# PKU-VCL-Geometry/GeoSplatting

Measured on AMD Instinct MI355X. Metric: fwd+bwd views/sec at 2M Gaussians, 800x800, higher is better.
Workload: dtype f32

## Files before the change

geosplatting_amd/csrc/gs_sort.hip:

```cpp
#include "gs_common.h"

#include <cstdlib>
#include <cstring>

#define RS_THREADS 256
#define RS_WAVES 4
#define RS_ITEMS 8
#define RS_TILE (RS_THREADS * RS_ITEMS)
#define RS_WCHUNK (64 * RS_ITEMS)

typedef unsigned long long u64;

static int tile_bits(int tile_w, int tile_h)
{
    unsigned n = (unsigned)(tile_w * tile_h);
    int b = 0;
    while (n > 1) { n >>= 1; ++b; }
    return b + 1;
}

struct PairItem { u64 key; int32_t val; };
struct PairIn {
    const u64* keys; const int32_t* vals;
    __device__ __forceinline__ PairItem load(int64_t i) const { return PairItem{ keys[i], vals[i] }; }
};
struct PairOut {
    u64* keys; int32_t* vals;
    __device__ __forceinline__ void store(int64_t i, const PairItem& it) const { keys[i] = it.key; vals[i] = it.val; }
};
struct PairDigit {
    int shift; unsigned mask;
    __device__ __forceinline__ unsigned operator()(const PairItem& it) const { return (unsigned)(it.key >> shift) & mask; }
};

struct U2In {
    const uint2* p;
    __device__ __forceinline__ uint2 load(int64_t i) const { return p[i]; }
};
struct U2Out {
    uint2* p;
    __device__ __forceinline__ void store(int64_t i, const uint2& it) const { p[i] = it; }
};
struct DepthIn {
    const float* depths;
    __device__ __forceinline__ uint2 load(int64_t i) const { return make_uint2(__float_as_uint(depths[i]), (unsigned)i); }
};
struct XDigit {
    int shift; unsigned mask;
    __device__ __forceinline__ unsigned operator()(const uint2& it) const { return (it.x >> shift) & mask; }
};
struct FinalTiles {
    int32_t* tile_ids; int32_t* flatten_ids;
    __device__ __forceinline__ void store(int64_t i, const uint2& it) const
    {
        flatten_ids[i] = (int32_t)it.y;
        tile_ids[i] = (int32_t)it.x;
    }
};
struct FinalOut {
    u64* isect_ids; int32_t* flatten_ids; const float* depths;
    __device__ __forceinline__ void store(int64_t i, const uint2& it) const
    {
        flatten_ids[i] = (int32_t)it.y;
        isect_ids[i] = ((u64)it.x << 32) | (u64)__float_as_uint(depths[it.y]);
    }
};

template <typename Item, typename In, typename Digit>
__global__ void __launch_bounds__(RS_THREADS)
radix_hist_kernel(GsCount nc, In in, Digit digit, int nbins, int nblocks, unsigned* __restrict__ table)
{
    const int64_t n = gs_count(nc);
    __shared__ unsigned hist[256];
    hist[threadIdx.x] = 0u;
    __syncthreads();
    const int64_t base = (int64_t)blockIdx.x * RS_TILE;
#pragma unroll 4
    for (int k = 0; k < RS_ITEMS; ++k) {
        const int64_t i = base + (int64_t)k * RS_THREADS + threadIdx.x;
        if (i < n) atomicAdd(&hist[digit(in.load(i))], 1u);
    }
    __syncthreads();
    if ((int)threadIdx.x < nbins) table[(size_t)threadIdx.x * nblocks + blockIdx.x] = hist[threadIdx.x];
}

__global__ void __launch_bounds__(256)
radix_rowscan_kernel(int nblocks, unsigned* __restrict__ table, unsigned* __restrict__ row_total)
{
    __shared__ unsigned wsum[4];
    unsigned* row = table + (size_t)blockIdx.x * nblocks;
    const int lane = threadIdx.x & 63, wave = threadIdx.x >> 6;
    unsigned carry = 0u;
    for (int i0 = 0; i0 < nblocks; i0 += 256) {
        const int i = i0 + threadIdx.x;
        const unsigned v = i < nblocks ? row[i] : 0u;
        unsigned incl = v;
        incl = gs_wave_incl_scan(incl);
        if (lane == 63) wsum[wave] = incl;
        __syncthreads();
        unsigned before = 0u, all = 0u;
        for (int w = 0; w < 4; ++w) { if (w < wave) before += wsum[w]; all += wsum[w]; }
        if (i < nblocks) row[i] = carry + before + incl - v;
        carry += all;
        __syncthreads();
    }
    if (threadIdx.x == 0) row_total[blockIdx.x] = carry;
}

template <typename Item, typename In, typename Digit, typename Out, int NBITS>
__global__ void __launch_bounds__(RS_THREADS)
radix_scatter_kernel(GsCount nc, In in, Digit digit, int nblocks, const unsigned* __restrict__ table,
                     const unsigned* __restrict__ row_total, Out out)
{
    const int64_t n = gs_count(nc);
    constexpr int NB = 1 << NBITS;
    __shared__ unsigned cnt[RS_WAVES][NB];
    __shared__ unsigned dstart[NB];
    __shared__ unsigned gbase[NB];
    __shared__ Item stage[RS_TILE];
    const int lane = threadIdx.x & 63, wave = threadIdx.x >> 6;
    for (int i = threadIdx.x; i < RS_WAVES * NB; i += RS_THREADS) (&cnt[0][0])[i] = 0u;
    __syncthreads();
    const int64_t bbase = (int64_t)blockIdx.x * RS_TILE;
    const int64_t wbase = bbase + (int64_t)wave * RS_WCHUNK;
    const int n_here = (n - bbase) < RS_TILE ? (int)((n - bbase) > 0 ? (n - bbase) : 0) : RS_TILE;
    const u64 lane_lt = (1ull << lane) - 1ull;
    Item item[RS_ITEMS];
    unsigned dig[RS_ITEMS];
    unsigned rank[RS_ITEMS];
#pragma unroll
    for (int k = 0; k < RS_ITEMS; ++k) {
        const int64_t i = wbase + (int64_t)k * 64 + lane;
        const bool valid = i < n;
        if (valid) item[k] = in.load(i);
        const unsigned d = valid ? digit(item[k]) : 0u;
        u64 m = __ballot(valid);
#pragma unroll
        for (int b = 0; b < NBITS; ++b) {
            const bool bit = (d >> b) & 1u;
            const u64 bal = __ballot(bit);
            m &= bit ? bal : ~bal;
        }
        const unsigned old = cnt[wave][d];
        __builtin_amdgcn_wave_barrier();
        const unsigned r = __popcll(m & lane_lt);
        if (valid && r == 0u) cnt[wave][d] = old + (unsigned)__popcll(m);
        __builtin_amdgcn_fence(__ATOMIC_RELEASE, "wavefront");
        __builtin_amdgcn_wave_barrier();
        __builtin_amdgcn_fence(__ATOMIC_ACQUIRE, "wavefront");
        dig[k] = d;
        rank[k] = old + r;
    }
    __syncthreads();
    {
        const int d = threadIdx.x;
        unsigned tot = 0u;
        if (d < NB) for (int w = 0; w < RS_WAVES; ++w) tot += cnt[w][d];
        unsigned incl = tot;
        incl = gs_wave_incl_scan(incl);
        __shared__ unsigned wtot[RS_WAVES];
        if (lane == 63) wtot[wave] = incl;
        __syncthreads();
        unsigned before = 0u;
        for (int w = 0; w < wave; ++w) before += wtot[w];
        if (d < NB) dstart[d] = before + incl - tot;
        __syncthreads();
        const unsigned rt = d < NB ? row_total[d] : 0u;
        unsigned rincl = rt;
        rincl = gs_wave_incl_scan(rincl);
        if (lane == 63) wtot[wave] = rincl;
        __syncthreads();
        unsigned rbefore = 0u;
        for (int w = 0; w < wave; ++w) rbefore += wtot[w];
        if (d < NB) gbase[d] = rbefore + rincl - rt + table[(size_t)d * nblocks + blockIdx.x];
    }
    __syncthreads();
#pragma unroll
    for (int k = 0; k < RS_ITEMS; ++k) {
        const int64_t i = wbase + (int64_t)k * 64 + lane;
        if (i < n) {
            const unsigned d = dig[k];
            unsigned off = dstart[d] + rank[k];
            for (int w = 0; w < wave; ++w) off += cnt[w][d];
            stage[off] = item[k];
        }
    }
    __syncthreads();
#pragma unroll 4
    for (int k = 0; k < RS_ITEMS; ++k) {
        const int p = k * RS_THREADS + (int)threadIdx.x;
        if (p < n_here) {
            const Item it = stage[p];
            const unsigned d = digit(it);
            out.store((int64_t)gbase[d] + (int64_t)(p - (int)dstart[d]), it);
        }
    }
}

template <typename Item, typename In, typename Digit, typename Out>
static int radix_pass(GsCount nc, In in, Digit digit, Out out, int nbits, unsigned* table, hipStream_t s)
{
    const int64_t n = nc.n;
    const int nblocks = (int)((n + RS_TILE - 1) / RS_TILE);
    const int nbins = 1 << nbits;
    unsigned* row_total = table + (size_t)256 * nblocks;
    hipLaunchKernelGGL((radix_hist_kernel<Item, In, Digit>), dim3(nblocks), dim3(RS_THREADS), 0, s, nc, in, digit, nbins, nblocks, table);
    GS_CHECK_LAUNCH();
    hipLaunchKernelGGL(radix_rowscan_kernel, dim3(nbins), dim3(256), 0, s, nblocks, table, row_total);
    GS_CHECK_LAUNCH();
    switch (nbits) {
#define RS_CASE(B) case B: hipLaunchKernelGGL((radix_scatter_kernel<Item, In, Digit, Out, B>), dim3(nblocks), dim3(RS_THREADS), 0, s, nc, in, digit, nblocks, table, row_total, out); break;
        RS_CASE(1) RS_CASE(2) RS_CASE(3) RS_CASE(4) RS_CASE(5) RS_CASE(6) RS_CASE(7) RS_CASE(8)
#undef RS_CASE
        default: gs_set_error("radix_pass: bad digit width %d", nbits); return GS_EINVAL;
    }
    GS_CHECK_LAUNCH();
    return GS_OK;
}

static size_t align256(size_t x) { return (x + 255) & ~(size_t)255; }
static size_t table_bytes(int64_t n) { return align256(((size_t)256 * (size_t)((n + RS_TILE - 1) / RS_TILE + 1) + 512) * sizeof(unsigned)); }

extern "C" size_t gs_sort_ws_bytes(int64_t n_isects, int tile_w, int tile_h)
{
    if (n_isects <= 0) return 0;
    (void)tile_w; (void)tile_h;
    return table_bytes(n_isects) + align256((size_t)n_isects * 8) + align256((size_t)n_isects * 4) + 256;
}

extern "C" int gs_isect_sort(int64_t n_isects, const int64_t* isect_ids, const int32_t* flatten_ids,
                             int64_t* isect_ids_sorted, int32_t* flatten_ids_sorted, int tile_w, int tile_h,
                             void* ws, size_t ws_bytes, void* stream)
{
    GS_CHECK_ARG(n_isects >= 0 && tile_w > 0 && tile_h > 0, "bad sizes");
    if (n_isects == 0) return GS_OK;
    GS_CHECK_ARG(ws != nullptr, "workspace must not be NULL");
    if (ws_bytes < gs_sort_ws_bytes(n_isects, tile_w, tile_h)) { gs_set_error("gs_isect_sort: workspace too small"); return GS_ENOSPC; }
    hipStream_t s = (hipStream_t)stream;
    char* p = (char*)ws;
    unsigned* table = (unsigned*)p; p += table_bytes(n_isects);
    u64* tk = (u64*)p; p += align256((size_t)n_isects * 8);
    int32_t* tv = (int32_t*)p;
    const int end_bit = 32 + tile_bits(tile_w, tile_h);
    const int npass = (end_bit + 7) / 8;
    const u64* src_k = (const u64*)isect_ids; const int32_t* src_v = flatten_ids;
    for (int pass = 0; pass < npass; ++pass) {
        const int shift = pass * 8;
        const int nbits = (end_bit - shift) < 8 ? (end_bit - shift) : 8;
        const bool to_out = ((npass - 1 - pass) % 2) == 0;
        u64* dk = to_out ? (u64*)isect_ids_sorted : tk;
        int32_t* dv = to_out ? flatten_ids_sorted : tv;
        const int rc = radix_pass<PairItem>(GsCount{ n_isects, nullptr }, PairIn{ src_k, src_v }, PairDigit{ shift, (1u << nbits) - 1u }, PairOut{ dk, dv }, nbits, table, s);
        if (rc != GS_OK) return rc;
        src_k = dk; src_v = dv;
    }
    return GS_OK;
}

__device__ __forceinline__ void tile_range_sorted(float mx, float my, int radius, int tile_size, int tw, int th,
                                                  int& x0, int& y0, int& x1, int& y1)
{
#pragma clang fp contract(off)
    const float ts = (float)tile_size;
    const float tr = (float)radius / ts;
    const float tx = mx / ts, ty = my / ts;
    const float fx0 = floorf(tx - tr), fy0 = floorf(ty - tr);
    const float fx1 = ceilf(tx + tr), fy1 = ceilf(ty + tr);
    x0 = fx0 < 0.0f ? 0 : (fx0 > (float)tw ? tw : (int)fx0);
    y0 = fy0 < 0.0f ? 0 : (fy0 > (float)th ? th : (int)fy0);
    x1 = fx1 < 0.0f ? 0 : (fx1 > (float)tw ? tw : (int)fx1);
    y1 = fy1 < 0.0f ? 0 : (fy1 > (float)th ? th : (int)fy1);
}

#define EM_THREADS 256
#define EM_PER 4
#define EM_LOOK 4
#define EM_TILE (EM_THREADS * EM_PER)

__global__ void __launch_bounds__(256)
tile_rect_kernel(GsCount vc, const float* __restrict__ means2d, const int32_t* __restrict__ radii, int tile_size, int tile_w, int tile_h,
                 uint2* __restrict__ rect)
{
    const int V = (int)gs_count(vc);
    const int v = blockIdx.x * blockDim.x + threadIdx.x;
    if (v >= V) return;
    const float2 m = *reinterpret_cast<const float2*>(means2d + 2 * (size_t)v);
    int x0 = 0, y0 = 0, x1 = 0, y1 = 0;
    const int r = radii[v];
    if (r > 0) tile_range_sorted(m.x, m.y, r, tile_size, tile_w, tile_h, x0, y0, x1, y1);
    rect[v] = make_uint2((unsigned)x0 | ((unsigned)y0 << 16), (unsigned)x1 | ((unsigned)y1 << 16));
}
__device__ __forceinline__ unsigned rect_count(uint2 q)
{
    const int w = (int)(q.y & 0xffffu) - (int)(q.x & 0xffffu), h = (int)(q.y >> 16) - (int)(q.x >> 16);
    return (w > 0 && h > 0) ? (unsigned)(w * h) : 0u;
}

static size_t bf_state_bytes(int V) { return align256(16 + 2 * (size_t)((V + EM_TILE - 1) / EM_TILE + 1) * sizeof(u64)); }

extern "C" size_t gs_isect_bin_ws_bytes(int V, int64_t n_isects, int tile_w, int tile_h)
{
    (void)tile_w; (void)tile_h;
    const size_t v = V > 0 ? (size_t)V : 1, n = n_isects > 0 ? (size_t)n_isects : 1;
    const size_t tb = table_bytes((int64_t)(v > n ? v : n));
    return tb + 3 * align256(v * 8) + bf_state_bytes((int)v) + 2 * align256(n * 8) + 256;
}

__global__ void capacity_check_kernel(const long long* __restrict__ counts, long long v_cap, long long i_cap, long long* __restrict__ status)
{
    if (threadIdx.x != 0 || blockIdx.x != 0) return;
    const long long V = counts[0], I = counts[1];
    if (V > v_cap || I > i_cap) {
        status[0] = GS_ENOSPC;
        if (I > status[1]) status[1] = I;
        if (V > status[2]) status[2] = V;
    }
}

static int isect_bin_impl(int V, const float* means2d, const int32_t* radii, const float* depths, int64_t n_isects,
                          const long long* counts_dev, int tile_size, int tile_w, int tile_h, int64_t* isect_ids_sorted,
                          int32_t* flatten_ids_sorted, void* ws, size_t ws_bytes, void* stream, int32_t* tile_ids_sorted);

extern "C" int gs_isect_bin(int V, const float* means2d, const int32_t* radii, const float* depths,
                            const int32_t* tiles_per_gauss, int64_t n_isects, int tile_size, int tile_w, int tile_h,
                            int64_t* isect_ids_sorted, int32_t* flatten_ids_sorted, void* ws, size_t ws_bytes, void* stream)
{
    (void)tiles_per_gauss;
    return isect_bin_impl(V, means2d, radii, depths, n_isects, nullptr, tile_size, tile_w, tile_h, isect_ids_sorted, flatten_ids_sorted,
                          ws, ws_bytes, stream, nullptr);
}

extern "C" int gs_isect_bin_cap(int V_cap, const float* means2d, const int32_t* radii, const float* depths, const int64_t* counts_dev,
                                int64_t n_isects_cap, int tile_size, int tile_w, int tile_h, int64_t* isect_ids_sorted,
                                int32_t* flatten_ids_sorted, void* ws, size_t ws_bytes, int64_t* status_dev, void* stream)
{
    GS_CHECK_ARG(counts_dev != nullptr && status_dev != nullptr, "counts_dev / status_dev must not be NULL");
    hipLaunchKernelGGL(capacity_check_kernel, dim3(1), dim3(64), 0, (hipStream_t)stream, (const long long*)counts_dev, (long long)V_cap,
                       (long long)n_isects_cap, (long long*)status_dev);
    GS_CHECK_LAUNCH();
    return isect_bin_impl(V_cap, means2d, radii, depths, n_isects_cap, (const long long*)counts_dev, tile_size, tile_w, tile_h,
                          isect_ids_sorted, flatten_ids_sorted, ws, ws_bytes, stream, nullptr);
}

extern "C" int gs_isect_bin_tiles_cap(int V_cap, const float* means2d, const int32_t* radii, const float* depths, const int64_t* counts_dev,
                                      int64_t n_isects_cap, int tile_size, int tile_w, int tile_h, int32_t* tile_ids_sorted,
                                      int32_t* flatten_ids_sorted, void* ws, size_t ws_bytes, int64_t* status_dev, void* stream)
{
    GS_CHECK_ARG(counts_dev != nullptr && status_dev != nullptr && tile_ids_sorted != nullptr, "counts_dev / status_dev / tile_ids_sorted must not be NULL");
    hipLaunchKernelGGL(capacity_check_kernel, dim3(1), dim3(64), 0, (hipStream_t)stream, (const long long*)counts_dev, (long long)V_cap,
                       (long long)n_isects_cap, (long long*)status_dev);
    GS_CHECK_LAUNCH();
    return isect_bin_impl(V_cap, means2d, radii, depths, n_isects_cap, (const long long*)counts_dev, tile_size, tile_w, tile_h,
                          nullptr, flatten_ids_sorted, ws, ws_bytes, stream, tile_ids_sorted);
}

struct KeyIn {
    const unsigned* keys;
    __device__ __forceinline__ uint2 load(int64_t i) const { return make_uint2(keys[i], (unsigned)i); }
};
struct FinalFlat {
    int32_t* flatten_ids;
    __device__ __forceinline__ void store(int64_t i, const uint2& it) const { flatten_ids[i] = (int32_t)it.y; }
};

#define BF_HIST_MAX 8192

__global__ void __launch_bounds__(256)
bin_setup_kernel(unsigned* __restrict__ state, int n_state_words,
                 const long long* __restrict__ counts, long long v_cap, long long i_cap, long long* __restrict__ status)
{
    const int i = blockIdx.x * blockDim.x + threadIdx.x, stride = gridDim.x * blockDim.x;
    for (int k = i; k < n_state_words; k += stride) state[k] = 0u;
    if (i == 0 && counts != nullptr && status != nullptr) {
        const long long V = counts[0], I = counts[1];
        if (V > v_cap || I > i_cap) {
            status[0] = GS_ENOSPC;
            if (I > status[1]) status[1] = I;
            if (V > status[2]) status[2] = V;
        }
    }
}

#define BF_VALID (1ull << 63)
#define BF_SPIN_LIMIT (1 << 22)

__global__ void __launch_bounds__(EM_THREADS)
emit_chained_kernel(GsCount vc, const uint2* __restrict__ order, const uint2* __restrict__ rect, unsigned* __restrict__ ctrl,
                    u64* __restrict__ desc, int n_blocks, int tile_w, uint2* __restrict__ items, unsigned item_cap,
                    long long* __restrict__ status )
{
    const int V = (int)gs_count(vc);
    __shared__ unsigned ws[EM_THREADS / 64];
    __shared__ unsigned s_block;
    __shared__ unsigned long long s_base;
    const int lane = threadIdx.x & 63, wave = threadIdx.x >> 6;
    if (threadIdx.x == 0) s_block = atomicAdd(ctrl, 1u);
    __syncthreads();
    const int block = (int)s_block;
    u64* agg = desc; u64* pre = desc + n_blocks;
    const int r0 = block * EM_TILE + (int)threadIdx.x * EM_PER;
    int v[EM_PER]; unsigned c[EM_PER]; uint2 q[EM_PER];
    unsigned mine = 0u;
#pragma unroll
    for (int k = 0; k < EM_PER; ++k) {
        const int r = r0 + k;
        v[k] = r < V ? (int)order[r].y : -1;
        q[k] = v[k] >= 0 ? rect[v[k]] : make_uint2(0u, 0u);
        c[k] = rect_count(q[k]);
        mine += c[k];
    }
    unsigned incl = mine;
    incl = gs_wave_incl_scan(incl);
    if (lane == 63) ws[wave] = incl;
    __syncthreads();
    unsigned before = 0u, total = 0u;
    for (int w = 0; w < EM_THREADS / 64; ++w) { if (w < wave) before += ws[w]; total += ws[w]; }
    if (wave == 0) {
        unsigned long long acc = 0ull;
        if (block > 0) {
            if (lane == 0) __hip_atomic_store(&agg[block], (u64)total | BF_VALID, __ATOMIC_RELAXED, __HIP_MEMORY_SCOPE_AGENT);
            int pos = block - 1;
            bool done = false;
            while (!done) {
                u64 pv[EM_LOOK], av[EM_LOOK];
#pragma unroll
                for (int j = 0; j < EM_LOOK; ++j) {
                    const int idx = pos - 64 * j - lane;
                    pv[j] = av[j] = 0ull;
                    if (idx >= 0) {
                        pv[j] = __hip_atomic_load(&pre[idx], __ATOMIC_RELAXED, __HIP_MEMORY_SCOPE_AGENT);
                        av[j] = __hip_atomic_load(&agg[idx], __ATOMIC_RELAXED, __HIP_MEMORY_SCOPE_AGENT);
                    }
                }
#pragma unroll
                for (int j = 0; j < EM_LOOK; ++j) {
                    if (done) break;
                    const int idx = pos - 64 * j - lane;
                    bool isP = idx < 0;
                    u64 val = 0ull;
                    if (idx >= 0) {
                        int spins = 0;
                        for (;;) {
                            if (pv[j] & BF_VALID) { isP = true; val = pv[j]; break; }
                            if (av[j] & BF_VALID) { val = av[j]; break; }
                            if (++spins > BF_SPIN_LIMIT) { atomicExch(ctrl + 1, 1u); if (status) status[0] = GS_ENOSPC; break; }
                            __builtin_amdgcn_s_sleep(2);
                            pv[j] = __hip_atomic_load(&pre[idx], __ATOMIC_RELAXED, __HIP_MEMORY_SCOPE_AGENT);
                            av[j] = __hip_atomic_load(&agg[idx], __ATOMIC_RELAXED, __HIP_MEMORY_SCOPE_AGENT);
                        }
                    }
                    const u64 pmask = __ballot(isP);
                    const int first = pmask ? __builtin_ctzll(pmask) : 64;
                    if (lane <= first) acc += val & ~BF_VALID;
                    if (pmask) done = true;
                }
                pos -= 64 * EM_LOOK;
            }
        }
        const unsigned long long base = gs_wave_sum_u64(acc);
        if (lane == 0) {
            __hip_atomic_store(&pre[block], (u64)(base + total) | BF_VALID, __ATOMIC_RELAXED, __HIP_MEMORY_SCOPE_AGENT);
            s_base = base;
        }
    }
    __syncthreads();
    unsigned long long cur = s_base + before + incl - mine;
#pragma unroll
    for (int k = 0; k < EM_PER; ++k) {
        if (v[k] < 0 || c[k] == 0u) continue;
        const int x0 = (int)(q[k].x & 0xffffu), y0 = (int)(q[k].x >> 16), x1 = (int)(q[k].y & 0xffffu), y1 = (int)(q[k].y >> 16);
        for (int i = y0; i < y1; ++i)
            for (int j = x0; j < x1; ++j) {
                const unsigned t = (unsigned)(i * tile_w + j);
                if (cur < (unsigned long long)item_cap) items[cur] = make_uint2(t, (unsigned)v[k]);
                ++cur;
            }
    }
}

__global__ void __launch_bounds__(1024)
tile_offsets_scan_kernel(int n_tiles, const unsigned* __restrict__ tile_counts, GsCount nc, int32_t* __restrict__ offsets)
{
    __shared__ unsigned wsum[16];
    const unsigned n = (unsigned)gs_count(nc);
    const int lane = threadIdx.x & 63, wave = threadIdx.x >> 6;
    unsigned carry = 0u;
    for (int i0 = 0; i0 < n_tiles; i0 += 1024) {
        const int i = i0 + threadIdx.x;
        const unsigned v = i < n_tiles ? tile_counts[i] : 0u;
        unsigned incl = v;
        incl = gs_wave_incl_scan(incl);
        if (lane == 63) wsum[wave] = incl;
        __syncthreads();
        unsigned before = 0u, all = 0u;
        for (int w = 0; w < 16; ++w) { if (w < wave) before += wsum[w]; all += wsum[w]; }
        if (i < n_tiles) { const unsigned o = carry + before + incl - v; offsets[i] = (int32_t)(o < n ? o : n); }
        carry += all;
        __syncthreads();
    }
}

__global__ void __launch_bounds__(256)
bin_offsets_tiles_kernel(GsCount nc, const int32_t* __restrict__ tiles, int n_tiles, int32_t* __restrict__ offsets)
{
    const int64_t n = gs_count(nc);
    const int64_t i = (int64_t)blockIdx.x * blockDim.x + threadIdx.x;
    if (n == 0 && i == 0)
        for (int t = 0; t < n_tiles; ++t) offsets[t] = 0;
    if (i >= n) return;
    const int cur = tiles[i];
    if (i == 0) {
        for (int t = 0; t <= cur && t < n_tiles; ++t) offsets[t] = 0;
    } else {
        const int prev = tiles[i - 1];
        for (int t = prev + 1; t <= cur && t < n_tiles; ++t) offsets[t] = (int32_t)i;
    }
    if (i == n - 1)
        for (int t = cur + 1; t < n_tiles; ++t) offsets[t] = (int32_t)n;
}


extern "C" size_t gs_isect_bin_front_ws_bytes(int V, int64_t n_isects, int tile_w, int tile_h)
{
    const size_t v = V > 0 ? (size_t)V : 1, n = n_isects > 0 ? (size_t)n_isects : 1;
    const size_t tb = table_bytes((int64_t)(v > n ? v : n));
    return tb + 2 * align256(v * 8) + 2 * align256(n * 8) + bf_state_bytes((int)v) + align256(n * 4) + 256;
}

extern "C" int gs_isect_bin_front(int V_cap, const uint32_t* depth_keys, const uint32_t* tile_rects, const uint32_t* tile_counts,
                                  const int64_t* counts_dev, int64_t n_isects_cap, int key_bits, int tile_w, int tile_h, int32_t* flatten_ids_sorted,
                                  int32_t* isect_offsets, void* ws, size_t ws_bytes, int64_t* status_dev, void* stream)
{
    const int V = V_cap;
    const int64_t n_isects = n_isects_cap;
    GS_CHECK_ARG(V >= 0 && n_isects >= 0 && tile_w > 0 && tile_h > 0 && (key_bits == 24 || key_bits == 32), "bad sizes or key width");
    GS_CHECK_ARG(n_isects < (1ll << 31), "n_isects must fit int32");
    GS_CHECK_ARG((int64_t)tile_w * tile_h < (1ll << 24) && tile_w < 65536 && tile_h < 65536, "tile grid too large");
    GS_CHECK_ARG(isect_offsets != nullptr && (counts_dev == nullptr || status_dev != nullptr), "null argument");
    hipStream_t s = (hipStream_t)stream;
    const int n_tiles = tile_w * tile_h;
    if (V == 0 || n_isects == 0) { GS_CHECK_HIP(gs_zero_async(isect_offsets, sizeof(int32_t) * (size_t)n_tiles, s)); return GS_OK; }
    GS_CHECK_ARG(depth_keys != nullptr && tile_rects != nullptr && flatten_ids_sorted != nullptr && ws != nullptr, "null argument");
    if (ws_bytes < gs_isect_bin_front_ws_bytes(V, n_isects, tile_w, tile_h)) { gs_set_error("gs_isect_bin_front: workspace too small"); return GS_ENOSPC; }
    const GsCount vc{ (long long)V, (const long long*)counts_dev }, ic{ (long long)n_isects, counts_dev ? (const long long*)counts_dev + 1 : nullptr };
    const bool hist = tile_counts != nullptr && n_tiles <= BF_HIST_MAX;
    char* p = (char*)ws;
    unsigned* table = (unsigned*)p; p += table_bytes((int64_t)V > n_isects ? (int64_t)V : n_isects);
    uint2* da = (uint2*)p; p += align256((size_t)V * 8);
    uint2* db = (uint2*)p; p += align256((size_t)V * 8);
    uint2* ia = (uint2*)p; p += align256((size_t)n_isects * 8);
    uint2* ib = (uint2*)p; p += align256((size_t)n_isects * 8);
    unsigned* state = (unsigned*)p; p += bf_state_bytes(V);
    int32_t* tile_ids = hist ? nullptr : (int32_t*)p;
    const int eblocks = (V + EM_TILE - 1) / EM_TILE;
    const int n_state_words = (int)(bf_state_bytes(V) / 4);
    hipLaunchKernelGGL(bin_setup_kernel, dim3(gs_cdiv(n_state_words, 256) < 64 ? gs_cdiv(n_state_words, 256) : 64),
                       dim3(256), 0, s, state, n_state_words, (const long long*)counts_dev,
                       (long long)V_cap, (long long)n_isects_cap, (long long*)status_dev);
    GS_CHECK_LAUNCH();
    int rc = radix_pass<uint2>(vc, KeyIn{ depth_keys }, XDigit{ 0, 255u }, U2Out{ da }, 8, table, s);
    if (rc != GS_OK) return rc;
    rc = radix_pass<uint2>(vc, U2In{ da }, XDigit{ 8, 255u }, U2Out{ db }, 8, table, s);
    if (rc != GS_OK) return rc;
    rc = radix_pass<uint2>(vc, U2In{ db }, XDigit{ 16, 255u }, U2Out{ da }, 8, table, s);
    if (rc != GS_OK) return rc;
    const uint2* order = da;
    if (key_bits == 32) {
        rc = radix_pass<uint2>(vc, U2In{ da }, XDigit{ 24, 255u }, U2Out{ db }, 8, table, s);
        if (rc != GS_OK) return rc;
        order = db;
    }
    unsigned* ctrl = state; u64* desc = (u64*)((char*)state + 16);
    hipLaunchKernelGGL(emit_chained_kernel, dim3(eblocks), dim3(EM_THREADS), 0, s, vc, order, (const uint2*)tile_rects, ctrl, desc,
                       eblocks + 1, tile_w, ia, (unsigned)n_isects, (long long*)status_dev);
    GS_CHECK_LAUNCH();
    if (hist) {
        hipLaunchKernelGGL(tile_offsets_scan_kernel, dim3(1), dim3(1024), 0, s, n_tiles, (const unsigned*)tile_counts, ic, isect_offsets);
        GS_CHECK_LAUNCH();
    }
    int tb = 0;
    while ((1 << tb) < n_tiles) ++tb;
    if (tb < 1) tb = 1;
    const int npass = (tb + 7) / 8, width = (tb + npass - 1) / npass;
    uint2* src = ia; uint2* dst = ib;
    for (int pass = 0; pass < npass; ++pass) {
        const int shift = pass * width;
        const int nbits = (tb - shift) < width ? (tb - shift) : width;
        if (pass == npass - 1 && hist)
            rc = radix_pass<uint2>(ic, U2In{ src }, XDigit{ shift, (1u << nbits) - 1u }, FinalFlat{ flatten_ids_sorted }, nbits, table, s);
        else if (pass == npass - 1)
            rc = radix_pass<uint2>(ic, U2In{ src }, XDigit{ shift, (1u << nbits) - 1u }, FinalTiles{ tile_ids, flatten_ids_sorted }, nbits, table, s);
        else
            rc = radix_pass<uint2>(ic, U2In{ src }, XDigit{ shift, (1u << nbits) - 1u }, U2Out{ dst }, nbits, table, s);
        if (rc != GS_OK) return rc;
        uint2* t = src; src = dst; dst = t;
    }
    if (!hist) {
        hipLaunchKernelGGL(bin_offsets_tiles_kernel, dim3(gs_cdiv(n_isects, 256)), dim3(256), 0, s, ic, tile_ids, n_tiles, isect_offsets);
        GS_CHECK_LAUNCH();
    }
    return GS_OK;
}

static int isect_bin_impl(int V, const float* means2d, const int32_t* radii, const float* depths, int64_t n_isects,
                          const long long* counts_dev, int tile_size, int tile_w, int tile_h, int64_t* isect_ids_sorted,
                          int32_t* flatten_ids_sorted, void* ws, size_t ws_bytes, void* stream, int32_t* tile_ids_sorted)
{
    const GsCount vc{ (long long)V, counts_dev }, ic{ (long long)n_isects, counts_dev ? counts_dev + 1 : nullptr };
    GS_CHECK_ARG(V >= 0 && n_isects >= 0 && tile_size > 0 && tile_w > 0 && tile_h > 0, "bad sizes");
    GS_CHECK_ARG(n_isects < (1ll << 31), "n_isects must fit int32");
    GS_CHECK_ARG((int64_t)tile_w * tile_h < (1ll << 24), "more than 2^24 tiles");
    if (V == 0 || n_isects == 0) return GS_OK;
    GS_CHECK_ARG(ws != nullptr, "workspace must not be NULL");
    if (ws_bytes < gs_isect_bin_ws_bytes(V, n_isects, tile_w, tile_h)) { gs_set_error("gs_isect_bin: workspace too small"); return GS_ENOSPC; }
    hipStream_t s = (hipStream_t)stream;
    char* p = (char*)ws;
    unsigned* table = (unsigned*)p; p += table_bytes((int64_t)V > n_isects ? (int64_t)V : n_isects);
    uint2* da = (uint2*)p; p += align256((size_t)V * 8);
    uint2* db = (uint2*)p; p += align256((size_t)V * 8);
    uint2* rect = (uint2*)p; p += align256((size_t)V * 8);
    const int eblocks = (V + EM_TILE - 1) / EM_TILE;
    unsigned* state = (unsigned*)p; p += bf_state_bytes(V);
    uint2* ia = (uint2*)p; p += align256((size_t)n_isects * 8);
    uint2* ib = (uint2*)p; p += align256((size_t)n_isects * 8);
    int tb = 0;
    while ((1 << tb) < tile_w * tile_h) ++tb;
    if (tb < 1) tb = 1;
    const int npass = (tb + 7) / 8, width = (tb + npass - 1) / npass;
    int rc = GS_OK;
    rc = radix_pass<uint2>(vc, DepthIn{ depths }, XDigit{ 0, 255u }, U2Out{ da }, 8, table, s);
    if (rc != GS_OK) return rc;
    rc = radix_pass<uint2>(vc, U2In{ da }, XDigit{ 8, 255u }, U2Out{ db }, 8, table, s);
    if (rc != GS_OK) return rc;
    rc = radix_pass<uint2>(vc, U2In{ db }, XDigit{ 16, 255u }, U2Out{ da }, 8, table, s);
    if (rc != GS_OK) return rc;
    rc = radix_pass<uint2>(vc, U2In{ da }, XDigit{ 24, 255u }, U2Out{ db }, 8, table, s);
    if (rc != GS_OK) return rc;
    GS_CHECK_ARG(tile_w < 65536 && tile_h < 65536, "tile grid too large");
    hipLaunchKernelGGL(tile_rect_kernel, dim3(gs_cdiv(V, 256)), dim3(256), 0, s, vc, means2d, radii, tile_size, tile_w, tile_h, rect);
    GS_CHECK_LAUNCH();
    {
        const int n_state_words = (int)(bf_state_bytes(V) / 4);
        hipLaunchKernelGGL(bin_setup_kernel, dim3(gs_cdiv(n_state_words, 256) < 64 ? gs_cdiv(n_state_words, 256) : 64), dim3(256), 0, s, state,
                           n_state_words, (const long long*)nullptr, 0ll, 0ll, (long long*)nullptr);
        GS_CHECK_LAUNCH();
        hipLaunchKernelGGL(emit_chained_kernel, dim3(eblocks), dim3(EM_THREADS), 0, s, vc, (const uint2*)db, (const uint2*)rect, state,
                           (u64*)((char*)state + 16), eblocks + 1, tile_w, ia, (unsigned)n_isects, (long long*)nullptr);
        GS_CHECK_LAUNCH();
    }
    uint2* src = ia; uint2* dst = ib;
    for (int pass = 0; pass < npass; ++pass) {
        const int shift = pass * width;
        const int nbits = (tb - shift) < width ? (tb - shift) : width;
        if (pass == npass - 1 && tile_ids_sorted != nullptr)
            rc = radix_pass<uint2>(ic, U2In{ src }, XDigit{ shift, (1u << nbits) - 1u },
                                   FinalTiles{ tile_ids_sorted, flatten_ids_sorted }, nbits, table, s);
        else if (pass == npass - 1)
            rc = radix_pass<uint2>(ic, U2In{ src }, XDigit{ shift, (1u << nbits) - 1u },
                                   FinalOut{ (u64*)isect_ids_sorted, flatten_ids_sorted, depths }, nbits, table, s);
        else
            rc = radix_pass<uint2>(ic, U2In{ src }, XDigit{ shift, (1u << nbits) - 1u }, U2Out{ dst }, nbits, table, s);
        if (rc != GS_OK) return rc;
        uint2* t = src; src = dst; dst = t;
    }
    return GS_OK;
}
```

Baseline: 724.3.

## Drop radix rowscan kernel via grouped histogram totals and fuse tile-offset scan

Removes the per-pass rowscan launch from the radix sort. The histogram kernel now writes a block-major table and atomically accumulates per-group (32 blocks) digit totals, and each scatter block computes its own global prefix from the group totals plus in-group block counts. The tile-offset scan is folded into the bin setup kernel as an extra block, and zeroing of the group buffers is merged into that setup. This saves one kernel launch per pass and its serial scan, at the cost of redundant prefix reads in every scatter block, global atomics in the histogram, and extra zeroing of workspace.

Result: no change. 723.0 (-0.2%).

```diff
diff --git a/geosplatting_amd/csrc/gs_sort.hip b/geosplatting_amd/csrc/gs_sort.hip
--- a/geosplatting_amd/csrc/gs_sort.hip
+++ b/geosplatting_amd/csrc/gs_sort.hip
@@ -8,6 +8,9 @@
 #define RS_ITEMS 8
 #define RS_TILE (RS_THREADS * RS_ITEMS)
 #define RS_WCHUNK (64 * RS_ITEMS)
+#define RS_GROUP_LOG2 5
+#define RS_GROUP (1 << RS_GROUP_LOG2)
+#define RS_MAX_PASSES 8
 
 typedef unsigned long long u64;
 
@@ -68,59 +71,60 @@
 
 template <typename Item, typename In, typename Digit>
 __global__ void __launch_bounds__(RS_THREADS)
-radix_hist_kernel(GsCount nc, In in, Digit digit, int nbins, int nblocks, unsigned* __restrict__ table)
+radix_hist_kernel(GsCount nc, In in, Digit digit, int nbins, unsigned* __restrict__ table, unsigned* __restrict__ gtot)
 {
     const int64_t n = gs_count(nc);
+    const int64_t base = (int64_t)blockIdx.x * RS_TILE;
+    if (base >= n) return;
     __shared__ unsigned hist[256];
     hist[threadIdx.x] = 0u;
     __syncthreads();
-    const int64_t base = (int64_t)blockIdx.x * RS_TILE;
 #pragma unroll 4
     for (int k = 0; k < RS_ITEMS; ++k) {
         const int64_t i = base + (int64_t)k * RS_THREADS + threadIdx.x;
         if (i < n) atomicAdd(&hist[digit(in.load(i))], 1u);
     }
     __syncthreads();
-    if ((int)threadIdx.x < nbins) table[(size_t)threadIdx.x * nblocks + blockIdx.x] = hist[threadIdx.x];
-}
-
-__global__ void __launch_bounds__(256)
-radix_rowscan_kernel(int nblocks, unsigned* __restrict__ table, unsigned* __restrict__ row_total)
-{
-    __shared__ unsigned wsum[4];
-    unsigned* row = table + (size_t)blockIdx.x * nblocks;
-    const int lane = threadIdx.x & 63, wave = threadIdx.x >> 6;
-    unsigned carry = 0u;
-    for (int i0 = 0; i0 < nblocks; i0 += 256) {
-        const int i = i0 + threadIdx.x;
-        const unsigned v = i < nblocks ? row[i] : 0u;
-        unsigned incl = v;
-        incl = gs_wave_incl_scan(incl);
-        if (lane == 63) wsum[wave] = incl;
-        __syncthreads();
-        unsigned before = 0u, all = 0u;
-        for (int w = 0; w < 4; ++w) { if (w < wave) before += wsum[w]; all += wsum[w]; }
-        if (i < nblocks) row[i] = carry + before + incl - v;
-        carry += all;
-        __syncthreads();
-    }
-    if (threadIdx.x == 0) row_total[blockIdx.x] = carry;
+    if ((int)threadIdx.x < nbins) {
+        const unsigned c = hist[threadIdx.x];
+        table[(size_t)blockIdx.x * nbins + threadIdx.x] = c;
+        if (c) atomicAdd(&gtot[(size_t)(blockIdx.x >> RS_GROUP_LOG2) * nbins + threadIdx.x], c);
+    }
 }
 
 template <typename Item, typename In, typename Digit, typename Out, int NBITS>
 __global__ void __launch_bounds__(RS_THREADS)
 radix_scatter_kernel(GsCount nc, In in, Digit digit, int nblocks, const unsigned* __restrict__ table,
-                     const unsigned* __restrict__ row_total, Out out)
+                     const unsigned* __restrict__ gtot, Out out)
 {
     const int64_t n = gs_count(nc);
+    if ((int64_t)blockIdx.x * RS_TILE >= n) return;
     constexpr int NB = 1 << NBITS;
     __shared__ unsigned cnt[RS_WAVES][NB];
     __shared__ unsigned dstart[NB];
     __shared__ unsigned gbase[NB];
     __shared__ Item stage[RS_TILE];
     const int lane = threadIdx.x & 63, wave = threadIdx.x >> 6;
+    unsigned* const dtotal = reinterpret_cast<unsigned*>(stage);
     for (int i = threadIdx.x; i < RS_WAVES * NB; i += RS_THREADS) (&cnt[0][0])[i] = 0u;
-    __syncthreads();
+    if ((int)threadIdx.x < NB) { gbase[threadIdx.x] = 0u; dtotal[threadIdx.x] = 0u; }
+    __syncthreads();
+    {
+        constexpr int PARTS = RS_THREADS / NB;
+        const int d = (int)threadIdx.x & (NB - 1), part = (int)threadIdx.x / NB;
+        const int g = (int)blockIdx.x >> RS_GROUP_LOG2, ngroups = (nblocks + RS_GROUP - 1) >> RS_GROUP_LOG2;
+        unsigned all = 0u, before = 0u;
+#pragma unroll 8
+        for (int k = part; k < ngroups; k += PARTS) {
+            const unsigned v = gtot[(size_t)k * NB + d];
+            all += v;
+            before += k < g ? v : 0u;
+        }
+#pragma unroll 8
+        for (int r = (g << RS_GROUP_LOG2) + part; r < (int)blockIdx.x; r += PARTS) before += table[(size_t)r * NB + d];
+        if (PARTS == 1) { dtotal[d] = all; gbase[d] = before; }
+        else { atomicAdd(&dtotal[d], all); atomicAdd(&gbase[d], before); }
+    }
     const int64_t bbase = (int64_t)blockIdx.x * RS_TILE;
     const int64_t wbase = bbase + (int64_t)wave * RS_WCHUNK;
     const int n_here = (n - bbase) < RS_TILE ? (int)((n - bbase) > 0 ? (n - bbase) : 0) : RS_TILE;
@@ -165,14 +169,14 @@
         for (int w = 0; w < wave; ++w) before += wtot[w];
         if (d < NB) dstart[d] = before + incl - tot;
         __syncthreads();
-        const unsigned rt = d < NB ? row_total[d] : 0u;
+        const unsigned rt = d < NB ? dtotal[d] : 0u;
         unsigned rincl = rt;
         rincl = gs_wave_incl_scan(rincl);
         if (lane == 63) wtot[wave] = rincl;
         __syncthreads();
         unsigned rbefore = 0u;
         for (int w = 0; w < wave; ++w) rbefore += wtot[w];
-        if (d < NB) gbase[d] = rbefore + rincl - rt + table[(size_t)d * nblocks + blockIdx.x];
+        if (d < NB) gbase[d] += rbefore + rincl - rt;
     }
     __syncthreads();
 #pragma unroll
@@ -198,18 +202,15 @@
 }
 
 template <typename Item, typename In, typename Digit, typename Out>
-static int radix_pass(GsCount nc, In in, Digit digit, Out out, int nbits, unsigned* table, hipStream_t s)
+static int radix_pass(GsCount nc, In in, Digit digit, Out out, int nbits, unsigned* table, unsigned* gtot, hipStream_t s)
 {
     const int64_t n = nc.n;
     const int nblocks = (int)((n + RS_TILE - 1) / RS_TILE);
     const int nbins = 1 << nbits;
-    unsigned* row_total = table + (size_t)256 * nblocks;
-    hipLaunchKernelGGL((radix_hist_kernel<Item, In, Digit>), dim3(nblocks), dim3(RS_THREADS), 0, s, nc, in, digit, nbins, nblocks, table);
-    GS_CHECK_LAUNCH();
-    hipLaunchKernelGGL(radix_rowscan_kernel, dim3(nbins), dim3(256), 0, s, nblocks, table, row_total);
+    hipLaunchKernelGGL((radix_hist_kernel<Item, In, Digit>), dim3(nblocks), dim3(RS_THREADS), 0, s, nc, in, digit, nbins, table, gtot);
     GS_CHECK_LAUNCH();
     switch (nbits) {
-#define RS_CASE(B) case B: hipLaunchKernelGGL((radix_scatter_kernel<Item, In, Digit, Out, B>), dim3(nblocks), dim3(RS_THREADS), 0, s, nc, in, digit, nblocks, table, row_total, out); break;
+#define RS_CASE(B) case B: hipLaunchKernelGGL((radix_scatter_kernel<Item, In, Digit, Out, B>), dim3(nblocks), dim3(RS_THREADS), 0, s, nc, in, digit, nblocks, table, gtot, out); break;
         RS_CASE(1) RS_CASE(2) RS_CASE(3) RS_CASE(4) RS_CASE(5) RS_CASE(6) RS_CASE(7) RS_CASE(8)
 #undef RS_CASE
         default: gs_set_error("radix_pass: bad digit width %d", nbits); return GS_EINVAL;
@@ -220,12 +221,14 @@
 
 static size_t align256(size_t x) { return (x + 255) & ~(size_t)255; }
 static size_t table_bytes(int64_t n) { return align256(((size_t)256 * (size_t)((n + RS_TILE - 1) / RS_TILE + 1) + 512) * sizeof(unsigned)); }
+static size_t group_words(int64_t n) { return (size_t)256 * (size_t)(((n + RS_TILE - 1) / RS_TILE + RS_GROUP - 1) / RS_GROUP + 1); }
+static size_t group_bytes(int64_t n) { return align256((size_t)RS_MAX_PASSES * group_words(n) * sizeof(unsigned)); }
 
 extern "C" size_t gs_sort_ws_bytes(int64_t n_isects, int tile_w, int tile_h)
 {
     if (n_isects <= 0) return 0;
     (void)tile_w; (void)tile_h;
-    return table_bytes(n_isects) + align256((size_t)n_isects * 8) + align256((size_t)n_isects * 4) + 256;
+    return table_bytes(n_isects) + group_bytes(n_isects) + align256((size_t)n_isects * 8) + align256((size_t)n_isects * 4) + 256;
 }
 
 extern "C" int gs_isect_sort(int64_t n_isects, const int64_t* isect_ids, const int32_t* flatten_ids,
@@ -239,10 +242,14 @@
     hipStream_t s = (hipStream_t)stream;
     char* p = (char*)ws;
     unsigned* table = (unsigned*)p; p += table_bytes(n_isects);
+    unsigned* groups = (unsigned*)p; p += group_bytes(n_isects);
     u64* tk = (u64*)p; p += align256((size_t)n_isects * 8);
     int32_t* tv = (int32_t*)p;
     const int end_bit = 32 + tile_bits(tile_w, tile_h);
     const int npass = (end_bit + 7) / 8;
+    GS_CHECK_ARG(npass <= RS_MAX_PASSES, "too many tiles");
+    const size_t gw = group_words(n_isects);
+    GS_CHECK_HIP(gs_zero_async(groups, (size_t)npass * gw * sizeof(unsigned), s));
     const u64* src_k = (const u64*)isect_ids; const int32_t* src_v = flatten_ids;
     for (int pass = 0; pass < npass; ++pass) {
         const int shift = pass * 8;
@@ -250,7 +257,7 @@
         const bool to_out = ((npass - 1 - pass) % 2) == 0;
         u64* dk = to_out ? (u64*)isect_ids_sorted : tk;
         int32_t* dv = to_out ? flatten_ids_sorted : tv;
-        const int rc = radix_pass<PairItem>(GsCount{ n_isects, nullptr }, PairIn{ src_k, src_v }, PairDigit{ shift, (1u << nbits) - 1u }, PairOut{ dk, dv }, nbits, table, s);
+        const int rc = radix_pass<PairItem>(GsCount{ n_isects, nullptr }, PairIn{ src_k, src_v }, PairDigit{ shift, (1u << nbits) - 1u }, PairOut{ dk, dv }, nbits, table, groups + (size_t)pass * gw, s);
         if (rc != GS_OK) return rc;
         src_k = dk; src_v = dv;
     }
@@ -274,7 +281,9 @@
 
 #define EM_THREADS 256
 #define EM_PER 4
+#ifndef EM_LOOK
 #define EM_LOOK 4
+#endif
 #define EM_TILE (EM_THREADS * EM_PER)
 
 __global__ void __launch_bounds__(256)
@@ -302,7 +311,7 @@
 {
     (void)tile_w; (void)tile_h;
     const size_t v = V > 0 ? (size_t)V : 1, n = n_isects > 0 ? (size_t)n_isects : 1;
-    const size_t tb = table_bytes((int64_t)(v > n ? v : n));
+    const size_t tb = table_bytes((int64_t)(v > n ? v : n)) + group_bytes((int64_t)(v > n ? v : n));
     return tb + 3 * align256(v * 8) + bf_state_bytes((int)v) + 2 * align256(n * 8) + 256;
 }
 
@@ -319,7 +328,8 @@
 
 static int isect_bin_impl(int V, const float* means2d, const int32_t* radii, const float* depths, int64_t n_isects,
                           const long long* counts_dev, int tile_size, int tile_w, int tile_h, int64_t* isect_ids_sorted,
-                          int32_t* flatten_ids_sorted, void* ws, size_t ws_bytes, void* stream, int32_t* tile_ids_sorted);
+                          int32_t* flatten_ids_sorted, void* ws, size_t ws_bytes, void* stream, int32_t* tile_ids_sorted,
+                          long long* status );
 
 extern "C" int gs_isect_bin(int V, const float* means2d, const int32_t* radii, const float* depths,
                             const int32_t* tiles_per_gauss, int64_t n_isects, int tile_size, int tile_w, int tile_h,
@@ -327,7 +337,7 @@
 {
     (void)tiles_per_gauss;
     return isect_bin_impl(V, means2d, radii, depths, n_isects, nullptr, tile_size, tile_w, tile_h, isect_ids_sorted, flatten_ids_sorted,
-                          ws, ws_bytes, stream, nullptr);
+                          ws, ws_bytes, stream, nullptr, nullptr);
 }
 
 extern "C" int gs_isect_bin_cap(int V_cap, const float* means2d, const int32_t* radii, const float* depths, const int64_t* counts_dev,
@@ -339,7 +349,7 @@
                        (long long)n_isects_cap, (long long*)status_dev);
     GS_CHECK_LAUNCH();
     return isect_bin_impl(V_cap, means2d, radii, depths, n_isects_cap, (const long long*)counts_dev, tile_size, tile_w, tile_h,
-                          isect_ids_sorted, flatten_ids_sorted, ws, ws_bytes, stream, nullptr);
+                          isect_ids_sorted, flatten_ids_sorted, ws, ws_bytes, stream, nullptr, (long long*)status_dev);
 }
 
 extern "C" int gs_isect_bin_tiles_cap(int V_cap, const float* means2d, const int32_t* radii, const float* depths, const int64_t* counts_dev,
@@ -351,7 +361,7 @@
                        (long long)n_isects_cap, (long long*)status_dev);
     GS_CHECK_LAUNCH();
     return isect_bin_impl(V_cap, means2d, radii, depths, n_isects_cap, (const long long*)counts_dev, tile_size, tile_w, tile_h,
-                          nullptr, flatten_ids_sorted, ws, ws_bytes, stream, tile_ids_sorted);
+                          nullptr, flatten_ids_sorted, ws, ws_bytes, stream, tile_ids_sorted, (long long*)status_dev);
 }
 
 struct KeyIn {
@@ -366,11 +376,33 @@
 #define BF_HIST_MAX 8192
 
 __global__ void __launch_bounds__(256)
-bin_setup_kernel(unsigned* __restrict__ state, int n_state_words,
-                 const long long* __restrict__ counts, long long v_cap, long long i_cap, long long* __restrict__ status)
-{
-    const int i = blockIdx.x * blockDim.x + threadIdx.x, stride = gridDim.x * blockDim.x;
+bin_setup_kernel(unsigned* __restrict__ state, int n_state_words, unsigned* __restrict__ groups, int n_group_words,
+                 const long long* __restrict__ counts, long long v_cap, long long i_cap, long long* __restrict__ status,
+                 int n_tiles, const unsigned* __restrict__ tile_counts , GsCount nc, int32_t* __restrict__ offsets)
+{
+    const int clear_blocks = (int)gridDim.x - (tile_counts != nullptr ? 1 : 0);
+    if ((int)blockIdx.x == clear_blocks) {
+        __shared__ unsigned wsum[4];
+        const unsigned n = (unsigned)gs_count(nc);
+        const int lane = threadIdx.x & 63, wave = threadIdx.x >> 6;
+        const int per = (n_tiles + 255) / 256, t0 = (int)threadIdx.x * per;
+        unsigned sum = 0u;
+        for (int k = 0; k < per; ++k) sum += t0 + k < n_tiles ? tile_counts[t0 + k] : 0u;
+        unsigned incl = sum;
+        incl = gs_wave_incl_scan(incl);
+        if (lane == 63) wsum[wave] = incl;
+        __syncthreads();
+        unsigned run = incl - sum;
+        for (int w = 0; w < wave; ++w) run += wsum[w];
+        for (int k = 0; k < per && t0 + k < n_tiles; ++k) {
+            offsets[t0 + k] = (int32_t)(run < n ? run : n);
+            run += tile_counts[t0 + k];
+        }
+        return;
+    }
+    const int i = blockIdx.x * blockDim.x + threadIdx.x, stride = clear_blocks * blockDim.x;
     for (int k = i; k < n_state_words; k += stride) state[k] = 0u;
+    for (int k = i; k < n_group_words; k += stride) groups[k] = 0u;
     if (i == 0 && counts != nullptr && status != nullptr) {
         const long long V = counts[0], I = counts[1];
         if (V > v_cap || I > i_cap) {
@@ -380,6 +412,8 @@
         }
     }
 }
+
+static int bin_setup_blocks(size_t words) { const int b = gs_cdiv((int64_t)words, 256); return b < 1 ? 1 : (b < 128 ? b : 128); }
 
 #define BF_VALID (1ull << 63)
 #define BF_SPIN_LIMIT (1 << 22)
@@ -478,28 +512,6 @@
     }
 }
 
-__global__ void __launch_bounds__(1024)
-tile_offsets_scan_kernel(int n_tiles, const unsigned* __restrict__ tile_counts, GsCount nc, int32_t* __restrict__ offsets)
-{
-    __shared__ unsigned wsum[16];
-    const unsigned n = (unsigned)gs_count(nc);
-    const int lane = threadIdx.x & 63, wave = threadIdx.x >> 6;
-    unsigned carry = 0u;
-    for (int i0 = 0; i0 < n_tiles; i0 += 1024) {
-        const int i = i0 + threadIdx.x;
-        const unsigned v = i < n_tiles ? tile_counts[i] : 0u;
-        unsigned incl = v;
-        incl = gs_wave_incl_scan(incl);
-        if (lane == 63) wsum[wave] = incl;
-        __syncthreads();
-        unsigned before = 0u, all = 0u;
-        for (int w = 0; w < 16; ++w) { if (w < wave) before += wsum[w]; all += wsum[w]; }
-        if (i < n_tiles) { const unsigned o = carry + before + incl - v; offsets[i] = (int32_t)(o < n ? o : n); }
-        carry += all;
-        __syncthreads();
-    }
-}
-
 __global__ void __launch_bounds__(256)
 bin_offsets_tiles_kernel(GsCount nc, const int32_t* __restrict__ tiles, int n_tiles, int32_t* __restrict__ offsets)
 {
@@ -523,7 +535,7 @@
 extern "C" size_t gs_isect_bin_front_ws_bytes(int V, int64_t n_isects, int tile_w, int tile_h)
 {
     const size_t v = V > 0 ? (size_t)V : 1, n = n_isects > 0 ? (size_t)n_isects : 1;
-    const size_t tb = table_bytes((int64_t)(v > n ? v : n));
+    const size_t tb = table_bytes((int64_t)(v > n ? v : n)) + group_bytes((int64_t)(v > n ? v : n));
     return tb + 2 * align256(v * 8) + 2 * align256(n * 8) + bf_state_bytes((int)v) + align256(n * 4) + 256;
 }
 
@@ -545,7 +557,9 @@
     const GsCount vc{ (long long)V, (const long long*)counts_dev }, ic{ (long long)n_isects, counts_dev ? (const long long*)counts_dev + 1 : nullptr };
     const bool hist = tile_counts != nullptr && n_tiles <= BF_HIST_MAX;
     char* p = (char*)ws;
-    unsigned* table = (unsigned*)p; p += table_bytes((int64_t)V > n_isects ? (int64_t)V : n_isects);
+    const int64_t n_max = (int64_t)V > n_isects ? (int64_t)V : n_isects;
+    unsigned* table = (unsigned*)p; p += table_bytes(n_max);
+    unsigned* groups = (unsigned*)p; p += group_bytes(n_max);
     uint2* da = (uint2*)p; p += align256((size_t)V * 8);
     uint2* db = (uint2*)p; p += align256((size_t)V * 8);
     uint2* ia = (uint2*)p; p += align256((size_t)n_isects * 8);
@@ -554,44 +568,45 @@
     int32_t* tile_ids = hist ? nullptr : (int32_t*)p;
     const int eblocks = (V + EM_TILE - 1) / EM_TILE;
     const int n_state_words = (int)(bf_state_bytes(V) / 4);
-    hipLaunchKernelGGL(bin_setup_kernel, dim3(gs_cdiv(n_state_words, 256) < 64 ? gs_cdiv(n_state_words, 256) : 64),
-                       dim3(256), 0, s, state, n_state_words, (const long long*)counts_dev,
-                       (long long)V_cap, (long long)n_isects_cap, (long long*)status_dev);
+    int tb = 0;
+    while ((1 << tb) < n_tiles) ++tb;
+    if (tb < 1) tb = 1;
+    const int npass = (tb + 7) / 8, width = (tb + npass - 1) / npass;
+    const int dpass = key_bits / 8;
+    const size_t gwv = group_words(V), gwi = group_words(n_isects);
+    const size_t n_group_words = (size_t)dpass * gwv + (size_t)npass * gwi;
+    hipLaunchKernelGGL(bin_setup_kernel, dim3(bin_setup_blocks(n_group_words > (size_t)n_state_words ? n_group_words : (size_t)n_state_words) + (hist ? 1 : 0)),
+                       dim3(256), 0, s, state, n_state_words, groups, (int)n_group_words, (const long long*)counts_dev,
+                       (long long)V_cap, (long long)n_isects_cap, (long long*)status_dev, n_tiles,
+                       hist ? (const unsigned*)tile_counts : (const unsigned*)nullptr, ic, isect_offsets);
     GS_CHECK_LAUNCH();
-    int rc = radix_pass<uint2>(vc, KeyIn{ depth_keys }, XDigit{ 0, 255u }, U2Out{ da }, 8, table, s);
+    int rc = radix_pass<uint2>(vc, KeyIn{ depth_keys }, XDigit{ 0, 255u }, U2Out{ da }, 8, table, groups, s);
     if (rc != GS_OK) return rc;
-    rc = radix_pass<uint2>(vc, U2In{ da }, XDigit{ 8, 255u }, U2Out{ db }, 8, table, s);
+    rc = radix_pass<uint2>(vc, U2In{ da }, XDigit{ 8, 255u }, U2Out{ db }, 8, table, groups + gwv, s);
     if (rc != GS_OK) return rc;
-    rc = radix_pass<uint2>(vc, U2In{ db }, XDigit{ 16, 255u }, U2Out{ da }, 8, table, s);
+    rc = radix_pass<uint2>(vc, U2In{ db }, XDigit{ 16, 255u }, U2Out{ da }, 8, table, groups + 2 * gwv, s);
     if (rc != GS_OK) return rc;
     const uint2* order = da;
     if (key_bits == 32) {
-        rc = radix_pass<uint2>(vc, U2In{ da }, XDigit{ 24, 255u }, U2Out{ db }, 8, table, s);
+        rc = radix_pass<uint2>(vc, U2In{ da }, XDigit{ 24, 255u }, U2Out{ db }, 8, table, groups + 3 * gwv, s);
         if (rc != GS_OK) return rc;
         order = db;
     }
+    unsigned* tgroups = groups + (size_t)dpass * gwv;
     unsigned* ctrl = state; u64* desc = (u64*)((char*)state + 16);
     hipLaunchKernelGGL(emit_chained_kernel, dim3(eblocks), dim3(EM_THREADS), 0, s, vc, order, (const uint2*)tile_rects, ctrl, desc,
                        eblocks + 1, tile_w, ia, (unsigned)n_isects, (long long*)status_dev);
     GS_CHECK_LAUNCH();
-    if (hist) {
-        hipLaunchKernelGGL(tile_offsets_scan_kernel, dim3(1), dim3(1024), 0, s, n_tiles, (const unsigned*)tile_counts, ic, isect_offsets);
-        GS_CHECK_LAUNCH();
-    }
-    int tb = 0;
-    while ((1 << tb) < n_tiles) ++tb;
-    if (tb < 1) tb = 1;
-    const int npass = (tb + 7) / 8, width = (tb + npass - 1) / npass;
     uint2* src = ia; uint2* dst = ib;
     for (int pass = 0; pass < npass; ++pass) {
         const int shift = pass * width;
         const int nbits = (tb - shift) < width ? (tb - shift) : width;
         if (pass == npass - 1 && hist)
-            rc = radix_pass<uint2>(ic, U2In{ src }, XDigit{ shift, (1u << nbits) - 1u }, FinalFlat{ flatten_ids_sorted }, nbits, table, s);
+            rc = radix_pass<uint2>(ic, U2In{ src }, XDigit{ shift, (1u << nbits) - 1u }, FinalFlat{ flatten_ids_sorted }, nbits, table, tgroups + (size_t)pass * gwi, s);
         else if (pass == npass - 1)
-            rc = radix_pass<uint2>(ic, U2In{ src }, XDigit{ shift, (1u << nbits) - 1u }, FinalTiles{ tile_ids, flatten_ids_sorted }, nbits, table, s);
+            rc = radix_pass<uint2>(ic, U2In{ src }, XDigit{ shift, (1u << nbits) - 1u }, FinalTiles{ tile_ids, flatten_ids_sorted }, nbits, table, tgroups + (size_t)pass * gwi, s);
         else
-            rc = radix_pass<uint2>(ic, U2In{ src }, XDigit{ shift, (1u << nbits) - 1u }, U2Out{ dst }, nbits, table, s);
+            rc = radix_pass<uint2>(ic, U2In{ src }, XDigit{ shift, (1u << nbits) - 1u }, U2Out{ dst }, nbits, table, tgroups + (size_t)pass * gwi, s);
         if (rc != GS_OK) return rc;
         uint2* t = src; src = dst; dst = t;
     }
@@ -604,7 +619,8 @@
 
 static int isect_bin_impl(int V, const float* means2d, const int32_t* radii, const float* depths, int64_t n_isects,
                           const long long* counts_dev, int tile_size, int tile_w, int tile_h, int64_t* isect_ids_sorted,
-                          int32_t* flatten_ids_sorted, void* ws, size_t ws_bytes, void* stream, int32_t* tile_ids_sorted)
+                          int32_t* flatten_ids_sorted, void* ws, size_t ws_bytes, void* stream, int32_t* tile_ids_sorted,
+                          long long* status )
 {
     const GsCount vc{ (long long)V, counts_dev }, ic{ (long long)n_isects, counts_dev ? counts_dev + 1 : nullptr };
     GS_CHECK_ARG(V >= 0 && n_isects >= 0 && tile_size > 0 && tile_w > 0 && tile_h > 0, "bad sizes");
@@ -615,7 +631,9 @@
     if (ws_bytes < gs_isect_bin_ws_bytes(V, n_isects, tile_w, tile_h)) { gs_set_error("gs_isect_bin: workspace too small"); return GS_ENOSPC; }
     hipStream_t s = (hipStream_t)stream;
     char* p = (char*)ws;
-    unsigned* table = (unsigned*)p; p += table_bytes((int64_t)V > n_isects ? (int64_t)V : n_isects);
+    const int64_t n_max = (int64_t)V > n_isects ? (int64_t)V : n_isects;
+    unsigned* table = (unsigned*)p; p += table_bytes(n_max);
+    unsigned* groups = (unsigned*)p; p += group_bytes(n_max);
     uint2* da = (uint2*)p; p += align256((size_t)V * 8);
     uint2* db = (uint2*)p; p += align256((size_t)V * 8);
     uint2* rect = (uint2*)p; p += align256((size_t)V * 8);
@@ -628,24 +646,30 @@
     if (tb < 1) tb = 1;
     const int npass = (tb + 7) / 8, width = (tb + npass - 1) / npass;
     int rc = GS_OK;
-    rc = radix_pass<uint2>(vc, DepthIn{ depths }, XDigit{ 0, 255u }, U2Out{ da }, 8, table, s);
+    const size_t gwv = group_words(V), gwi = group_words(n_isects);
+    unsigned* tgroups = groups + 4 * gwv;
+    {
+        const int n_state_words = (int)(bf_state_bytes(V) / 4);
+        const size_t n_group_words = 4 * gwv + (size_t)npass * gwi;
+        hipLaunchKernelGGL(bin_setup_kernel, dim3(bin_setup_blocks(n_group_words > (size_t)n_state_words ? n_group_words : (size_t)n_state_words)),
+                           dim3(256), 0, s, state, n_state_words, groups, (int)n_group_words, (const long long*)nullptr, 0ll, 0ll,
+                           (long long*)nullptr, 0, (const unsigned*)nullptr, ic, (int32_t*)nullptr);
+        GS_CHECK_LAUNCH();
+    }
+    rc = radix_pass<uint2>(vc, DepthIn{ depths }, XDigit{ 0, 255u }, U2Out{ da }, 8, table, groups, s);
     if (rc != GS_OK) return rc;
-    rc = radix_pass<uint2>(vc, U2In{ da }, XDigit{ 8, 255u }, U2Out{ db }, 8, table, s);
+    rc = radix_pass<uint2>(vc, U2In{ da }, XDigit{ 8, 255u }, U2Out{ db }, 8, table, groups + gwv, s);
     if (rc != GS_OK) return rc;
-    rc = radix_pass<uint2>(vc, U2In{ db }, XDigit{ 16, 255u }, U2Out{ da }, 8, table, s);
+    rc = radix_pass<uint2>(vc, U2In{ db }, XDigit{ 16, 255u }, U2Out{ da }, 8, table, groups + 2 * gwv, s);
     if (rc != GS_OK) return rc;
-    rc = radix_pass<uint2>(vc, U2In{ da }, XDigit{ 24, 255u }, U2Out{ db }, 8, table, s);
+    rc = radix_pass<uint2>(vc, U2In{ da }, XDigit{ 24, 255u }, U2Out{ db }, 8, table, groups + 3 * gwv, s);
     if (rc != GS_OK) return rc;
     GS_CHECK_ARG(tile_w < 65536 && tile_h < 65536, "tile grid too large");
     hipLaunchKernelGGL(tile_rect_kernel, dim3(gs_cdiv(V, 256)), dim3(256), 0, s, vc, means2d, radii, tile_size, tile_w, tile_h, rect);
     GS_CHECK_LAUNCH();
     {
-        const int n_state_words = (int)(bf_state_bytes(V) / 4);
-        hipLaunchKernelGGL(bin_setup_kernel, dim3(gs_cdiv(n_state_words, 256) < 64 ? gs_cdiv(n_state_words, 256) : 64), dim3(256), 0, s, state,
-                           n_state_words, (const long long*)nullptr, 0ll, 0ll, (long long*)nullptr);
-        GS_CHECK_LAUNCH();
         hipLaunchKernelGGL(emit_chained_kernel, dim3(eblocks), dim3(EM_THREADS), 0, s, vc, (const uint2*)db, (const uint2*)rect, state,
-                           (u64*)((char*)state + 16), eblocks + 1, tile_w, ia, (unsigned)n_isects, (long long*)nullptr);
+                           (u64*)((char*)state + 16), eblocks + 1, tile_w, ia, (unsigned)n_isects, status);
         GS_CHECK_LAUNCH();
     }
     uint2* src = ia; uint2* dst = ib;
@@ -654,12 +678,12 @@
         const int nbits = (tb - shift) < width ? (tb - shift) : width;
         if (pass == npass - 1 && tile_ids_sorted != nullptr)
             rc = radix_pass<uint2>(ic, U2In{ src }, XDigit{ shift, (1u << nbits) - 1u },
-                                   FinalTiles{ tile_ids_sorted, flatten_ids_sorted }, nbits, table, s);
+                                   FinalTiles{ tile_ids_sorted, flatten_ids_sorted }, nbits, table, tgroups + (size_t)pass * gwi, s);
         else if (pass == npass - 1)
             rc = radix_pass<uint2>(ic, U2In{ src }, XDigit{ shift, (1u << nbits) - 1u },
-                                   FinalOut{ (u64*)isect_ids_sorted, flatten_ids_sorted, depths }, nbits, table, s);
+                                   FinalOut{ (u64*)isect_ids_sorted, flatten_ids_sorted, depths }, nbits, table, tgroups + (size_t)pass * gwi, s);
         else
-            rc = radix_pass<uint2>(ic, U2In{ src }, XDigit{ shift, (1u << nbits) - 1u }, U2Out{ dst }, nbits, table, s);
+            rc = radix_pass<uint2>(ic, U2In{ src }, XDigit{ shift, (1u << nbits) - 1u }, U2Out{ dst }, nbits, table, tgroups + (size_t)pass * gwi, s);
         if (rc != GS_OK) return rc;
         uint2* t = src; src = dst; dst = t;
     }
```
